# mpieva/mapAD

Measured on AMD Instinct MI355X. Metric: mapped reads/sec (50 bp, -p 0.03), higher is better.
Workload: dtype u64+f32; 1 GPU; C4: synthetic genome (3000000000 bp, n = 6000000002 BWT rows), 10000000 x 50 bp reads per GPU, -p 0.03, no-damage model; reads_per_gpu=10000000, genome_bp=3000000000, index_bytes_hbm=3000000128, batches_in_flight=2, parallelism=1 GPU, index_build=GPU suffix sorting (prefix doubling over radix sorts) + host text preparation

## Files before the change

mapad_amd/csrc/darray_core.hpp:

```cpp
#pragma once
#include "search_core.hpp"

namespace mapad {

constexpr int kMaxOffset = 15;

MAPAD_HD float d_penalty(const DevParams& P, const uint8_t* seq, const uint8_t* qual, int L, int r) {
    const int to_class = base_index(seq[r]);
    const Float4 row = sdm_row(P, L, r, qual[r], to_class);
    float v = sdm_best_mismatch(row, to_class) - sdm_optimal(row, to_class);
    const int dist = r < (L - r - 1) ? r : (L - r - 1);
    if (dist >= P.gap_dist_ends) v = f32_max(v, P.gap_extend);
    return v;
}

MAPAD_HD void ext1_any(const DevIndex& ix, uint64_t lower, uint64_t size, int k, int w, uint64_t& nl, uint64_t& ns) {
#if defined(__HIP_DEVICE_COMPILE__)
    ext1_quad(ix, lower, size, k, w, nl, ns);
#else
    (void)w;
    ext1_scalar(ix, lower, size, k, nl, ns);
#endif
}

MAPAD_HD uint32_t d_chain(const DevIndex& ix, const uint8_t* seq, int L, int split, bool left_part, int offset, const float* pen,
                          float* out, int w) {
    const int part_len = left_part ? split : L - split;
    for (int p = 0; p <= offset && p < part_len; ++p) out[p] = 0.0f;
    float z = 0.0f, m = kF32Min;
    uint64_t lower = 0, size = ix.n;
    uint32_t n_ext = 0;
    for (int i = offset; i + 1 < part_len; ++i) {
        const int r = left_part ? i : L - 1 - i;
        m = f32_max(m, pen[r]);
        const int b = base_index(seq[r]);
        uint64_t nl = 0, ns = 0;
        if (b < 4) ext1_any(ix, lower, size, left_part ? 3 - b : b, w, nl, ns);
        n_ext += 1;
        if (ns < 1) {
            z += m;
            m = kF32Min;
            lower = 0; size = ix.n;
        } else {
            lower = nl; size = ns;
        }
        out[i + 1] = z;
    }
    return n_ext;
}

MAPAD_HD uint32_t d_array_scalar(const DevIndex& ix, const DevParams& P, const uint8_t* seq, const uint8_t* qual, int L, float* pen_buf,
                                 float* chain_buf, float* d_out) {
    const int split = P.start_at_end ? L : L / 2;
    for (int r = 0; r < L; ++r) { pen_buf[r] = d_penalty(P, seq, qual, L, r); d_out[r] = 0.0f; }
    uint32_t n_ext = 0;
    for (int part = 0; part < 2; ++part) {
        const bool left = part == 0;
        const int part_len = left ? split : L - split;
        for (int o = 0; o < kMaxOffset; ++o) {
            n_ext += d_chain(ix, seq, L, split, left, o, pen_buf, chain_buf, 0);
            for (int p = 0; p < part_len; ++p) {
                float& d = d_out[(left ? 0 : split) + p];
                d = f32_min(d, chain_buf[p]);
            }
        }
    }
    return n_ext;
}

}
```

mapad_amd/csrc/mapad_amd.hip:

```cpp
#include <hip/hip_runtime.h>

#include <algorithm>
#include <atomic>
#include <cstdio>
#include <cstdlib>
#include <cstring>
#include <map>
#include <memory>
#include <mutex>
#include <new>
#include <set>
#include <stdexcept>
#include <string>
#include <type_traits>
#include <unordered_map>
#include <vector>

#include "../../include/mapad_amd.h"
#include "collapse_core.hpp"
#include "darray_core.hpp"
#include "host_index.hpp"
#include "host_index_io.hpp"
#include "host_models.hpp"
#include "host_postproc.hpp"
#include "postproc_core.hpp"
#include "text_core.hpp"
#include "damage_core.hpp"
#include "coverage_core.hpp"
#include "pileup_core.hpp"
#include "panel_core.hpp"
#include "allele_core.hpp"
#include "genotype_core.hpp"
#include "dedup_core.hpp"
#include "dscore_core.hpp"
#include "rescale_core.hpp"
#include "align_core.hpp"
#include "merge_core.hpp"
#include "mappability_core.hpp"
#include "search_core.hpp"
#include "host_tail.hpp"

using namespace mapad;

namespace mapad { namespace gpuidx { void suffix_products(const uint8_t* t_host, host::Index& ix, int device, bool verbose); void last_build_info(uint64_t out[16]); } }

namespace {

enum : uint32_t { ST_POOL_OVERFLOW = 4, ST_NO_TABLE = 8, ST_TAIL = 16  };
#if !defined(MAPAD_DEFAULT_TAIL_POPS)
#define MAPAD_DEFAULT_TAIL_POPS (1u << 20)
#endif
#if !defined(MAPAD_DEFAULT_TAIL_POPS_IDLE)
#define MAPAD_DEFAULT_TAIL_POPS_IDLE (1u << 17)
#endif
constexpr int kTiers = 2;
constexpr int kStages = 3;
constexpr int kClasses = 10;
constexpr int kKeyBins = kMaxReadLen + 2;
enum { CUR_HITS = 0, CUR_OPS = 2, CUR_POOL_OVF = 4, CUR_ERR = 5, CUR_WORK = 6, CUR_OVF = 7, CUR_GROWN = 6 + 2 * kStages, CUR_HEAVY_N = CUR_GROWN + 4 , CUR_HEAVY_WORK = CUR_GROWN + 6 ,
       CUR_HEAVY_POPS = CUR_GROWN + 8 , CUR_HPROF = CUR_GROWN + 10 , CUR_TAIL = CUR_GROWN + 26 , CUR_TAIL_DRY = CUR_GROWN + 27 ,
       CUR_TAIL_F = CUR_GROWN + 28 , CUR_TAIL_STATE = CUR_GROWN + 29 ,
       CUR_TAIL_IDLE = CUR_GROWN + 30 , CUR_COUNT = CUR_GROWN + 31 };
inline uint64_t cur64(const uint32_t* cur, int k) { return (uint64_t)cur[k] | ((uint64_t)cur[k + 1] << 32); }

struct BatchDev {
    const uint8_t* seqs;
    const uint8_t* quals;
    const uint64_t* offsets;
    uint32_t n_reads;
    float* d_arrays;
    ReadCounters* counters;
    uint32_t* status;
    uint32_t* hit_count;
    uint32_t* hit_first;
    HitRec* hits_pool;
    uint32_t* ops_pool;
    uint32_t hits_cap, ops_cap;
    uint32_t* cursors;
    uint32_t* overflow_list;
    uint32_t* sort_key;
    uint32_t* key_hist;
    uint32_t order_shift;
    uint32_t* order;
    unsigned long long* prof;
    struct HeavyItem* heavy;
    uint32_t heavy_cap;
    uint8_t* tail_ring;
    uint32_t tail_stride, tail_cap, tail_lmax;
    uint32_t tail_pops;
    const uint32_t* tail_ctl;
    uint32_t tail_backlog_max, tail_min_class;
    uint32_t tail_backlog_budget;
    uint32_t tail_continue;
    uint32_t tail_gen;
    uint32_t tail_pops_idle, tail_backlog_idle;
};

struct HeavyItem {
    uint32_t read, grown;
    SearchState st;
};
static_assert(sizeof(HeavyItem) == 72, "heavy item layout");

struct ArenaPool {
    uint8_t* base;
    uint64_t stride;
    uint64_t off_nodes, off_hits, off_hit_ops, off_scratch, off_near;
    uint32_t heap_cap, node_cap, hit_ops_cap;
    uint32_t* set_owner;
    uint32_t n_sets;
};

struct GrowPools {
    uint8_t* base[kClasses + 1];
    uint32_t* owner[kClasses + 1];
    uint64_t stride[kClasses + 1], off_nodes[kClasses + 1];
    uint64_t off_hits[kClasses + 1], off_hit_ops[kClasses + 1], off_scratch[kClasses + 1];
    uint32_t heap_cap[kClasses + 1], node_cap[kClasses + 1], count[kClasses + 1];
    uint32_t set_next_class;
    uint32_t hit_ops_cap;
    uint32_t max_waits;
    uint32_t heavy_min_class;
    uint32_t wide_copy_nodes;
    uint32_t heavy_fast;
    uint32_t heavy_max_pending;
};
constexpr uint32_t kGrownShift = 27;

template <bool NL, int TOP = kTop>
__device__ __forceinline__ ArenaT<NL, TOP> carve(const ArenaPool& ap, uint32_t slot) {
    uint8_t* b = ap.base + (uint64_t)slot * ap.stride;
    ArenaT<NL, TOP> a;
    a.heap = (MAPAD_GLOBAL HeapEntry*)(b) + 1;
    a.nodes = (MAPAD_GLOBAL Node*)(b + ap.off_nodes);
    a.hits = (MAPAD_GLOBAL HitRec*)(b + ap.off_hits);
    a.hit_ops = (MAPAD_GLOBAL uint32_t*)(b + ap.off_hit_ops);
    a.scratch = (MAPAD_GLOBAL uint16_t*)(b + ap.off_scratch);
    a.top = nullptr;
    a.heap_cap = ap.heap_cap; a.node_cap = ap.node_cap; a.hit_ops_cap = ap.hit_ops_cap;
    return a;
}

#define MAPAD_SLIM_EARLY __launch_bounds__(64)
__global__ void MAPAD_SLIM_EARLY darray_kernel(DevIndex ix, DevParams P, BatchDev B, int lmax, float* long_scratch, const uint32_t* __restrict__ dup_of) {
    extern __shared__ float lds[];
    float* pen = long_scratch ? long_scratch + (size_t)blockIdx.x * 16 * lmax : lds;
    float* chains = pen + lmax;
    __shared__ uint32_t n_ext_total;
    const int lane = threadIdx.x & 63, quad = lane >> 2, w = lane & 3;
    for (uint32_t read = blockIdx.x; read < B.n_reads; read += gridDim.x) {
        if (dup_of && dup_of[read] != read) continue;
        const uint64_t off = B.offsets[read];
        const int L = (int)(B.offsets[read + 1] - off);
        const uint8_t* seq = B.seqs + off;
        const uint8_t* qual = B.quals + off;
        float* dout = B.d_arrays + off;
        if (L > lmax || P.table_base[L] < 0) {
            if (lane == 0) {
                B.status[read] = ST_NO_TABLE; atomicOr(&B.cursors[CUR_ERR], ST_NO_TABLE); B.counters[read].e_darray = 0;
                if (B.order) { B.sort_key[read] = 0; atomicAdd(&B.key_hist[(size_t)(read >> B.order_shift) * kKeyBins], 1u); }
            }
            continue;
        }
        const int split = P.start_at_end ? L : L / 2;
        uint32_t zeros = 0;
        if (lane == 0) n_ext_total = 0;
        for (int r = lane; r < L; r += 64) pen[r] = d_penalty(P, seq, qual, L, r);
        __syncthreads();
        for (int part = 0; part < 2; ++part) {
            const bool left = part == 0;
            const int part_len = left ? split : L - split;
            if (part_len == 0) continue;
            if (quad < kMaxOffset) {
                const uint32_t n_ext = d_chain(ix, seq, L, split, left, quad, pen, chains + quad * lmax, w);
                if (w == 0) atomicAdd(&n_ext_total, n_ext);
            }
            __syncthreads();
            for (int p = lane; p < part_len; p += 64) {
                float acc = 0.0f;
#pragma unroll
                for (int o = 0; o < kMaxOffset; ++o) acc = f32_min(acc, chains[o * lmax + p]);
                dout[(left ? 0 : split) + p] = acc;
                zeros += (uint32_t)__popcll(__ballot(acc == 0.0f));
            }
            __syncthreads();
        }
        if (lane == 0) {
            B.counters[read].e_darray = n_ext_total;
            if (B.order) { B.sort_key[read] = zeros; atomicAdd(&B.key_hist[(size_t)(read >> B.order_shift) * kKeyBins + zeros], 1u); }
        }
        __syncthreads();
    }
}

__global__ void order_scan_kernel(uint32_t* hist, uint32_t n_chunks, uint32_t n_bins, const uint32_t* first) {
    if (threadIdx.x != 0 || blockIdx.x != 0) return;
    uint32_t acc = first ? *first : 0u;
    for (uint32_t ch = 0; ch < n_chunks; ++ch) {
        uint32_t* h = hist + (size_t)ch * kKeyBins;
        for (int k = (int)n_bins - 1; k >= 0; --k) { const uint32_t c = h[k]; h[k] = acc; acc += c; }
    }
}
#define MAPAD_SLIM __launch_bounds__(64)
__global__ void MAPAD_SLIM order_scatter_kernel(BatchDev B, const uint32_t* __restrict__ dup_of) {
    const uint32_t lane = threadIdx.x & 63u;
    const uint32_t i = blockIdx.x * 64u + lane;
    const bool act = i < B.n_reads && (!dup_of || dup_of[i] == i);
    const uint32_t key = act ? B.sort_key[i] : 0xFFFFFFFFu;
    uint32_t* hist = B.key_hist + (size_t)((blockIdx.x * 64u) >> B.order_shift) * kKeyBins;
    uint64_t todo = __ballot(act);
    while (todo) {
        const int leader = __ffsll((long long)todo) - 1;
        const uint32_t k = (uint32_t)__builtin_amdgcn_readlane((int)key, leader);
        const bool mine = act && key == k;
        const uint64_t m = __ballot(mine);
        uint32_t base = 0;
        if ((int)lane == leader) base = atomicAdd(&hist[k], (uint32_t)__popcll(m));
        base = (uint32_t)__builtin_amdgcn_readlane((int)base, leader);
        if (mine) B.order[base + (uint32_t)__popcll(m & ((1ull << lane) - 1ull))] = i;
        todo &= ~m;
    }
}

enum { CS_GROUPS = 0, CS_TWIN_REPS = 1, CS_COLLISIONS = 2, CS_LIST = 3, CS_POPS = 4 , CS_COUNT = 8 };
struct CollapseDev {
    const uint8_t* seqs; const uint8_t* quals; const uint64_t* offsets;
    uint32_t n_reads, ignore_qual;
    collapse::Table tab;
    uint64_t* keys;
    uint32_t* dup_of;
    uint32_t* has_dup;
    uint32_t* stats;
};
struct CollapseAtomics {
    static __device__ __forceinline__ uint64_t cas64(uint64_t* p, uint64_t expected, uint64_t desired) { return (uint64_t)atomicCAS((unsigned long long*)p, (unsigned long long)expected, (unsigned long long)desired); }
    static __device__ __forceinline__ void max32(uint32_t* p, uint32_t v) { atomicMax(p, v); }
};
__global__ void MAPAD_SLIM collapse_insert_kernel(CollapseDev Q) {
    const uint32_t lane = threadIdx.x & 63u, w = lane & 3u;
    const uint32_t i = blockIdx.x * 16u + (lane >> 2);
    const bool act = i < Q.n_reads;
    uint64_t part = 0;
    int L = 0;
    if (act) {
        const uint64_t off = Q.offsets[i];
        L = (int)(Q.offsets[i + 1] - off);
        part = collapse::key_partial(Q.seqs + off, Q.quals + off, L, Q.ignore_qual != 0, (int)w, 4);
    }
    part += __shfl_xor(part, 1); part += __shfl_xor(part, 2);
    if (act && w == 0) {
        const uint64_t key = collapse::key_finish(part, L);
        Q.keys[i] = key;
        collapse::table_insert<CollapseAtomics>(Q.tab, key, i);
    }
}
__global__ void MAPAD_SLIM collapse_match_kernel(CollapseDev Q) {
    const uint32_t lane = threadIdx.x & 63u, w = lane & 3u;
    const uint32_t i = blockIdx.x * 16u + (lane >> 2);
    const bool act = i < Q.n_reads;
    uint32_t cand = i;
    bool same = true;
    if (act) {
        cand = collapse::table_find(Q.tab, Q.keys[i], i);
        if (cand != i) {
            const uint64_t off = Q.offsets[i], off_c = Q.offsets[cand];
            const int L = (int)(Q.offsets[i + 1] - off);
            same = (int)(Q.offsets[cand + 1] - off_c) == L &&
                   collapse::equal_partial(Q.seqs + off, Q.quals + off, Q.seqs + off_c, Q.quals + off_c, L, Q.ignore_qual != 0, (int)w, 4);
        }
    }
    const uint64_t agree = __ballot(same);
    same = ((agree >> (lane & ~3u)) & 0xFull) == 0xFull;
// ... 1372 lines not shown

#if !defined(MAPAD_KTOP2)
#define MAPAD_KTOP2 31
#endif
template <int LPR> struct top_of { static constexpr int value = LPR == 2 ? MAPAD_KTOP2 : kTop; };
template <int LPR, bool CONT, int PASS, bool NL, bool HEAVY, bool BWD = false>
__global__ void __launch_bounds__(64, (LPR == 1 && NL) ? 1 : LPR == 2 ? 2 : MAPAD_MIN_WAVES) search_kernel(DevIndex ix, DevParams P, BatchDev B0, ArenaPool AP0, const GrowPools* GP, uint32_t near_stride, uint32_t near_lmax, int stage) {
    const int lane = threadIdx.x & 63, w0 = lane & (LPR - 1);
    const int tier0 = stage;
    const uint32_t n_items = tier0 == 0 ? B0.n_reads : B0.cursors[CUR_OVF + 2 * (tier0 - 1)];
    if (n_items == 0) return;
    uint32_t* const cursors = B0.cursors;
    const uint32_t set = acquire_set(AP0);
    const uint32_t slot = set * (64 / LPR) + (lane / LPR);
    constexpr int TOPK = top_of<LPR>::value;
    static_assert(!HEAVY || LPR == 4, "reads are handed to heavy wavefronts by quads only");
    static_assert(!BWD || (LPR == 4 && !HEAVY), "the backward-only step is built for the default quads only");
    ArenaT<NL, TOPK> A = carve<NL, TOPK>(AP0, slot);
    extern __shared__ __attribute__((aligned(16))) uint8_t near_lds[];
    using NearBytes = typename near_ptr<uint8_t, NL>::type;
    NearBytes near;
    if constexpr (NL) near = (NearBytes)near_lds + (size_t)(lane / LPR) * near_stride;
    else near = AP0.base + (uint64_t)slot * AP0.stride + AP0.off_near;
    A.top = (typename near_ptr<HeapEntry, NL>::type)near + 1;
    const NearBytes near_qc = near + (TOPK + 1) * sizeof(HeapEntry);
    const typename near_ptr<float, NL>::type near_d = (typename near_ptr<float, NL>::type)(near_qc + ((2 * near_lmax + 15) & ~15u));
    uint32_t* work = &cursors[CUR_WORK + 2 * tier0];
    const DeviceGrow<LPR, NL, TOPK> grow{GP, &cursors[CUR_GROWN], slot, w0, stage + 2 < kStages || HEAVY, false, B0.tail_min_class};
    const uint32_t wide_copy_nodes = GP->wide_copy_nodes;
    const uint32_t tail_lo = B0.tail_pops_idle;
    bool tail_denied = false;
    bool drained = false;
#if defined(MAPAD_PROFILE_SECTIONS)
    if (lane < 2 * PROF_N + 2) g_prof_lds[lane] = 0;
    g_prof_hist[lane] = 0;
    if (lane == 0) g_prof_lds[2 * PROF_N] = __builtin_amdgcn_s_memtime();
#endif
    bool have = false, done = false;
    ReadInT<NL> rd{near_qc, near_d, 0, 0.0f, 0};
    if constexpr (LPR == 4) rd.lane_less = w0 == 0 ? ix.less[1] : w0 == 1 ? ix.less[2] : w0 == 2 ? ix.less[3] : ix.less[4];
    if constexpr (LPR == 2) { rd.lane_less = w0 == 0 ? ix.less[1] : ix.less[3]; rd.lane_less1 = w0 == 0 ? ix.less[2] : ix.less[4]; }
    SearchState st;
#if MAPAD_NODE_PREFETCH
    NodePrefetch node_pf;
#endif
    uint32_t read = 0;
    for (;;) {
        int w = w0, tier = tier0;
#if MAPAD_OPAQUE_LANE
        asm volatile("" : "+v"(w));
        asm volatile("" : "+s"(tier));
#endif
        MAPAD_MARK(PROF_LOOP);
        if (!have && !done) {
            uint32_t item = 0;
            if (w == 0 && !drained) item = atomicAdd(work, 1u);
            item = group_bcast<LPR>(item);
            uint32_t again = ~0u;
            if (PASS == 0 && !HEAVY && (drained | (item >= n_items))) {
                drained = true;
                if (w == 0) {
                    const uint32_t cnt = __hip_atomic_load(&cursors[CUR_OVF], __ATOMIC_RELAXED, __HIP_MEMORY_SCOPE_AGENT);
                    uint32_t cur = __hip_atomic_load(&cursors[CUR_WORK + 2], __ATOMIC_RELAXED, __HIP_MEMORY_SCOPE_AGENT);
                    while (cur < cnt) {
                        const uint32_t old = atomicCAS(&cursors[CUR_WORK + 2], cur, cur + 1u);
                        if (old == cur) { again = cur; break; }
                        cur = old;
                    }
                }
                again = group_bcast<LPR>(again);
            }
            if ((item >= n_items || drained) && again == ~0u) done = true;
            else {
                const BatchDev B = kernarg_reload(kArgOffB, B0);
                const uint32_t* items = B.overflow_list + (size_t)(tier > 0 ? tier - 1 : 0) * B.n_reads;
                if (again != ~0u) {
                    uint32_t e = 0;
                    if (w == 0) { while ((e = atomicExch(&B.overflow_list[again], 0u)) == 0u) __builtin_amdgcn_s_sleep(8); }
                    read = group_bcast<LPR>(e) - 1u;
                } else {
                    read = tier == 0 ? (B.order ? B.order[item] : item) : items[item] - 1u;
                    if (tier >= 1 && w == 0) B.overflow_list[(size_t)(tier - 1) * B.n_reads + item] = 0u;
                }
                const uint64_t off = B.offsets[read];
                rd.L = (int)(B.offsets[read + 1] - off);
                const DevParams Pf = kernarg_reload(kArgOffP, P);
                rd.thr = Pf.reject_thr[rd.L];
                rd.table = Pf.table_base[rd.L];
                if (tier == 0 && B.status[read] == ST_NO_TABLE) {
                    if (w == 0) { B.hit_count[read] = 0; B.hit_first[read] = 0; }
                } else {
                    read_setup(B.seqs + off, B.quals + off, B.d_arrays + off, rd.L, near_qc, near_d, w, LPR);
                    SearchState tmp;
                    A.n_waits = again != ~0u ? kRestarted : 0u;
                    search_init(kernarg_reload(0, ix).n, BWD ? rd.L : alignment_start_of(P, rd.L), rd, A, tmp);
                    st = tmp;
#if MAPAD_NODE_PREFETCH
                    node_pf.ok = false;
#endif
                    have = true;
                    tail_denied = false;
                }
                drain_memory();
            }
        }
        MAPAD_MARK(PROF_SETUP);
        if (__all(done)) break;
        if constexpr (PASS != 1 && LPR == 4) {
            const bool need = have && (st.heap_len != 0) & (st.status == ST_OK) & ((st.tree_len + kStepNodes > A.node_cap) | (st.heap_len + kStepNodes > A.heap_cap)) &
                              (st.tree_entries >= wide_copy_nodes);
            if (MAPAD_UNLIKELY(__any(need))) { grow.wide(A, st, lane, need); drain_memory(); }
        }
        if (have) {
            bool cont;
            DevParams Ps = P;
#if MAPAD_OPAQUE_LANE
            if constexpr (BWD) asm volatile("" : "+s"(Ps.nq), "+s"(Ps.bound_kind), "+s"(Ps.gap_dist_ends), "+s"(Ps.max_num_gaps_open), "+s"(Ps.stack_limit_abort));
            else asm volatile("" : "+s"(Ps.nq), "+s"(Ps.bound_kind), "+s"(Ps.gap_dist_ends), "+s"(Ps.max_num_gaps_open), "+s"(Ps.start_at_end), "+s"(Ps.stack_limit_abort));
#endif
#if MAPAD_NODE_PREFETCH
            if constexpr (PASS != 1 && LPR == 4 && NL) cont = search_step_pf<LPR, CONT, NL, false, BWD>(ix, Ps, rd, A, st, w, grow, node_pf);
            else
#endif
            if constexpr (PASS != 1) cont = search_step<LPR, CONT, NL, false, BWD>(ix, Ps, rd, A, st, w, grow);
            else cont = search_step<LPR, CONT, NL, false, BWD>(ix, Ps, rd, A, st, w, NoGrow());
            MAPAD_MARK(PROF_TAIL);
            auto give_to_host = [&](int why, uint32_t limit) -> int {
                const BatchDev B = kernarg_reload(kArgOffB, B0);
                if (B.tail_cap == 0) return 2;
                uint32_t k = 0xFFFFFFFEu;
                if (w == 0) {
                    if (limit == 0xFFFFFFFFu) k = atomicAdd(&cursors[CUR_TAIL], 1u);
                    else {
                        const uint32_t seen = __hip_atomic_load(B.tail_ctl + 1, __ATOMIC_RELAXED, __HIP_MEMORY_SCOPE_SYSTEM);
                        const uint32_t pend = __hip_atomic_load(B.tail_ctl, __ATOMIC_RELAXED, __HIP_MEMORY_SCOPE_SYSTEM);
                        uint32_t cur = __hip_atomic_load(&cursors[CUR_TAIL], __ATOMIC_RELAXED, __HIP_MEMORY_SCOPE_AGENT);
                        for (;;) {
                            if (cur >= B.tail_cap) { k = 0xFFFFFFFFu; break; }
                            if ((uint64_t)pend + (cur > seen ? cur - seen : 0u) >= limit) break;
                            const uint32_t old = atomicCAS(&cursors[CUR_TAIL], cur, cur + 1u);
                            if (old == cur) { k = cur; break; }
                            cur = old;
                        }
                    }
                }
                k = group_bcast<LPR>(k);
                if (k >= B.tail_cap) return k == 0xFFFFFFFEu ? 1 : 2;
                const bool with_state = PASS != 1 && TOPK == kTop && B.tail_continue != 0 && A.grown != 0 && st.n_hits == 0 && st.status == ST_OK;
                hand_to_host<LPR, NL>(B, rd, A, st, read, k, w, with_state);
                if (w == 0 && why) atomicAdd(&cursors[why], 1u);
                if (with_state) {
                    if (w == 0) atomicAdd(&cursors[CUR_TAIL_STATE], 1u);
                    const ArenaT<NL, TOPK> base = carve<NL, TOPK>(kernarg_reload(kArgOffAP, AP0), slot);
                    A.heap = base.heap; A.nodes = base.nodes; A.heap_cap = base.heap_cap; A.node_cap = base.node_cap; A.grown = 0;
                }
                return 0;
            };
// ... 169 lines not shown
    ArenaPool ap{};
    auto align = [](uint64_t x) { return (x + 127) & ~127ull; };
    ap.heap_cap = heap_cap; ap.node_cap = node_cap; ap.hit_ops_cap = hit_ops_cap;
    uint64_t o = align(heap_bytes(heap_cap));
    ap.off_nodes = o; o = align(o + (uint64_t)node_cap * sizeof(Node));
    ap.off_hits = o; o = align(o + (uint64_t)kMaxHits * sizeof(HitRec));
    ap.off_hit_ops = o; o = align(o + (uint64_t)hit_ops_cap * 4);
    ap.off_scratch = o; o = align(o + 2ull * (lmax + 1) * 2);
    ap.off_near = o; o = align(o + near_bytes(lmax));
    ap.stride = o;
    return ap;
}

}

namespace {
int zero_async(hipStream_t st, void* p, size_t bytes) {
    const uint64_t n = bytes / 4;
    if (!n) return MAPAD_OK;
    const uint32_t grid = (uint32_t)std::min<uint64_t>((n + 255) / 256, 4096);
    hipLaunchKernelGGL(zero_words_kernel, dim3(grid), dim3(64), 0, st, (uint32_t*)p, n);
    HIP_TRY(hipGetLastError());
    return MAPAD_OK;
}
int read_back_words(hipStream_t st, const void* d_src, PinnedBuf<uint32_t>& h, size_t word_off, uint32_t n_words) {
    hipLaunchKernelGGL(publish_words_kernel, dim3(1), dim3(64), 0, st, (const uint32_t*)d_src, h.data() + word_off, n_words);
    HIP_TRY(hipGetLastError());
    HIP_TRY(hipStreamSynchronize(st));
    return MAPAD_OK;
}
}

constexpr int kMaxDepth = 16;
enum Stage { ST_DEDUP, ST_DSCORE, ST_RESCALE, ST_DAMAGE, ST_COVERAGE, ST_PILEUP, ST_ALLELE, ST_GENOTYPE, ST_PANEL, ST_COUNT };
struct SlotStage {
    uint64_t gen = 0;
    DevEvent ev[2];
    bool untimed = false;
};
struct StageSums {
    uint64_t batches = 0;
    double ms = 0.0;
};
struct BatchSlot {
    hipStream_t stream = nullptr;
    bool own_stream = false;
    DevEvent ev[4];
    DevEvent ev_in;
    DevBuf<uint8_t> d_seqs, d_quals;
    DevBuf<uint64_t> d_offsets;
    DevBuf<float> d_darr, d_dscratch;
    DevBuf<ReadCounters> d_counters;
    DevBuf<uint32_t> d_status, d_hit_count, d_hit_first, d_ops, d_cursors, d_overflow, d_sort_key, d_key_hist, d_order;
    DevBuf<HitRec> d_hits;
    DevBuf<HeavyItem> d_heavy;
    DevBuf<uint64_t> d_c_hit_begin, d_c_ops_begin;
    DevBuf<unsigned long long> d_c_tiles;
    DevBuf<HitRec> d_c_hits;
    DevBuf<uint32_t> d_c_ops;
    uint64_t c_n_hits = 0, c_n_ops = 0;
    bool compacted = false;
    BatchDev last{};
    uint64_t last_total_bases = 0;
    uint32_t last_lmax = 0;
    uint32_t launch_info[8] = {0, 0, 0, 0, 0, 0, 0, 0};
    bool ev_valid = false, timed = true;
    uint64_t gen = 0;
    CoherentBuf tail_ring;
    uint32_t tail_ring_stride = 0, tail_ring_gen = 0;
    const uint8_t* tail_ring_base = nullptr;
    std::shared_ptr<std::atomic<bool>> tail_launched;
    bool tail_failed = false;
    std::shared_ptr<host::TailBatch> tail;
    DevBuf<uint8_t> d_tail_up;
    PinnedBuf<uint32_t> h_small;
    PinnedBuf<uint8_t> h_tail_stage;
    DevBuf<CoordRec> d_rec_coords;
    DevBuf<DevRecord> d_rec_out;
    DevBuf<char> d_rec_text;
    DevBuf<float> d_rec_pairs;
    DevBuf<uint32_t> d_dup_of, d_c_zeroed;
    DevBuf<uint64_t> d_c_keys;
    DevEvent ev_c[4];
    bool collapsed = false, fan_done = false, fan_d = false;
    uint32_t* c_stats = nullptr;
    SlotStage st[ST_COUNT];
    DevBuf<uint64_t> d_dd_keys;
    DevBuf<uint8_t> d_dup;
    DevBuf<int32_t> d_ds_score;
    DevBuf<uint8_t> d_ds_scored, d_ds_skip;
    DevBuf<uint8_t> d_rs_quals;
    DevBuf<AlignIn> d_an_in;
    DevBuf<uint32_t> d_an_cigar;
    DevBuf<uint8_t> d_an_md, d_an_cls;
    bool aligned = false;
    uint64_t tail_info[16] = {};

    void release() {
        d_seqs.release(); d_quals.release(); d_offsets.release(); d_darr.release(); d_dscratch.release(); d_counters.release(); d_status.release(); d_hit_count.release();
        d_hit_first.release(); d_ops.release(); d_cursors.release(); d_overflow.release(); d_sort_key.release(); d_key_hist.release(); d_order.release();
        d_hits.release(); d_heavy.release();
        d_c_hit_begin.release(); d_c_ops_begin.release(); d_c_tiles.release(); d_c_hits.release(); d_c_ops.release();
        if (tail) { host::tail_cancel(tail); tail.reset(); }
        d_tail_up.release();
        d_dup_of.release(); d_c_zeroed.release(); d_c_keys.release(); c_stats = nullptr; collapsed = false;
        for (auto& e : ev_c) e.reset();
        for (auto& s : st) { for (auto& e : s.ev) e.reset(); s.untimed = false; s.gen = 0; }
        d_dd_keys.release(); d_dup.release(); d_ds_score.release(); d_ds_scored.release(); d_ds_skip.release(); d_rs_quals.release();
        d_an_in.release(); d_an_cigar.release(); d_an_md.release(); d_an_cls.release(); aligned = false;
        d_rec_coords.release(); d_rec_out.release(); d_rec_text.release(); d_rec_pairs.release();
        for (auto& e : ev) e.reset(); ev_in.reset();
        if (own_stream && stream) (void)hipStreamDestroy(stream);
        stream = nullptr; own_stream = false;
    }
};

struct PanelDef {
    std::vector<uint64_t> slot_x;
    std::vector<uint32_t> slot_of_row;
    std::vector<uint8_t> alleles;
    bool operator==(const PanelDef& o) const { return slot_x == o.slot_x && slot_of_row == o.slot_of_row && alleles == o.alleles; }
};

struct mapad_ctx {
    int device = 0;
    hipStream_t stream = nullptr;
    mapad_params_t params{};
    const mapad_index* index = nullptr;
    host::HostTables tables;
    bool tables_dirty = true;
    std::shared_ptr<const host::HostTables> tables_snap;
    uint32_t tail_pops = 0;
    DevBuf<uint64_t> d_blocks;
    DevBuf<float> d_sdm, d_thr;
    DevBuf<int32_t> d_base;
    DevIndex dix{};
    DevParams dprm{};
    bool fetch_d = true;
    bool collapse = false;
    StageSums st[ST_COUNT];
    DevEvent ev_sum[2];
    int damage_mode = 0;
    DevBuf<unsigned long long> d_damage;
    int coverage_mode = 0;
    DevBuf<int32_t> d_cov_diff;
    DevBuf<unsigned long long> d_cov_cnt;
    DevBuf<uint32_t> d_cov_flag;
    DevBuf<CoverageSeg> d_cov_segs;
    DevBuf<long long> d_cov_sums;
    uint32_t cov_seg = 0;
    uint64_t cov_n_segs = 0;
    DevBuf<uint32_t> d_cov_win;
    DevBuf<int32_t> d_cov_tmp;
// ... 638 lines not shown
    HIP_TRY(hipStreamCreateWithFlags(out, hipStreamNonBlocking));
    return MAPAD_OK;
}

void drop_tail(mapad_ctx* c, BatchSlot& S);
int acquire_slot(mapad_ctx* c, int k) {
    BatchSlot& S = c->bs[k];
    if (S.ev_valid) { HIP_TRY(hipStreamSynchronize(S.stream)); int rc = record_times(c, S); if (rc) return rc; }
    drop_tail(c, S);
    if (c->depth == 1) S.stream = c->stream;
    else if (!S.stream) { const int rc_s = create_slot_stream(c, &S.stream); if (rc_s) return rc_s; S.own_stream = true; }
    if (c->depth > 1) {
        if (S.ev_in.ensure(hipEventDisableTiming)) return MAPAD_ERR_DEVICE;
        HIP_TRY(hipEventRecord(S.ev_in, c->stream));
        HIP_TRY(hipStreamWaitEvent(S.stream, S.ev_in, 0));
    }
    c->cur = k; c->view = k;
    return MAPAD_OK;
}

uint32_t order_shift_for(uint64_t n_reads) {
    return std::min<uint32_t>(std::max<uint32_t>(env_u32("MAPAD_ORDER_CHUNK_LOG2", n_reads >= (4u << 20) ? 21 : 20), 10), 31);
}

uint64_t collapse_table_slots(uint64_t n_reads) { uint64_t t = 64; while (t < 2 * n_reads) t <<= 1; return t; }
size_t collapse_zeroed_words(uint64_t n_reads) { return (size_t)CS_COUNT + (size_t)((n_reads + 1) & ~1ull) + 3 * (size_t)collapse_table_slots(n_reads); }

int ensure_batch_buffers(mapad_ctx* c, BatchSlot& S, uint64_t n_reads, uint64_t total_bases, uint32_t lmax, bool host_inputs) {
    int rc;
    if ((rc = upload_tables(c))) return rc;
    if ((rc = ensure_arenas(c, S, lmax, n_reads))) return rc;
    const size_t nr = std::max<uint64_t>(n_reads, 1);
    if (host_inputs) {
        if ((rc = S.d_seqs.ensure(std::max<uint64_t>(total_bases, 1)))) return rc;
        if ((rc = S.d_quals.ensure(std::max<uint64_t>(total_bases, 1)))) return rc;
        if ((rc = S.d_offsets.ensure(n_reads + 1))) return rc;
    }
    if ((rc = S.d_darr.ensure(std::max<uint64_t>(total_bases, 1)))) return rc;
    if ((rc = S.d_counters.ensure(nr))) return rc;
    if ((rc = S.d_status.ensure(nr))) return rc;
    if ((rc = S.d_hit_count.ensure(nr))) return rc;
    if ((rc = S.d_hit_first.ensure(nr))) return rc;
    {
        const uint32_t* before = S.d_overflow.p;
        if ((rc = S.d_overflow.ensure(nr * kStages))) return rc;
        if (S.d_overflow.p != before) HIP_TRY(hipMemsetAsync(S.d_overflow.p, 0, S.d_overflow.cap * sizeof(uint32_t), S.stream));
    }
    const uint32_t order_shift = order_shift_for(nr);
    const uint32_t n_chunks = (uint32_t)((nr + (1ull << order_shift) - 1) >> order_shift);
    if (env_u32("MAPAD_ORDER", 1) != 0) {
        if ((rc = S.d_sort_key.ensure(nr))) return rc;
        if ((rc = S.d_order.ensure(nr))) return rc;
        if ((rc = S.d_key_hist.ensure((size_t)n_chunks * kKeyBins))) return rc;
    }
    if (c->collapse) {
        if ((rc = S.d_order.ensure(nr))) return rc;
        if ((rc = S.d_dup_of.ensure(nr))) return rc;
        if ((rc = S.d_c_keys.ensure(nr))) return rc;
        if ((rc = S.d_c_zeroed.ensure(collapse_zeroed_words(nr)))) return rc;
    }
    if ((rc = S.d_cursors.ensure(CUR_COUNT))) return rc;
    if ((rc = S.d_heavy.ensure(2 * (size_t)c->heavy_cap))) return rc;
    const size_t hits_cap = std::max(S.d_hits.cap, (size_t)env_u32("MAPAD_HIT_POOL", (uint32_t)std::min<size_t>(2 * nr + 1024, 0xFFFFFFFFu)));
    const size_t ops_cap = std::max(S.d_ops.cap, hits_cap * (size_t)(std::min<uint32_t>(lmax, 256) + 8));
    if ((rc = S.d_hits.ensure(hits_cap))) return rc;
    if ((rc = S.d_ops.ensure(ops_cap))) return rc;
    return MAPAD_OK;
}

bool release_tail_arena(mapad_ctx* c, uint32_t grown, hipStream_t st) {
    const uint32_t cls = (grown >> kGrownShift) - 1, idx = grown & ((1u << kGrownShift) - 1);
    if (cls > (uint32_t)kClasses || idx >= c->grow.count[cls]) return false;
    hipLaunchKernelGGL(zero_words_kernel, dim3(1), dim3(64), 0, st, c->grow.owner[cls] + idx, (uint64_t)1);
    return hipGetLastError() == hipSuccess;
}
hipStream_t thread_stream(int dev) {
    static thread_local hipStream_t streams[16] = {};
    if (dev < 0 || dev >= 16) return nullptr;
    if (!streams[dev] && hipStreamCreateWithFlags(&streams[dev], hipStreamNonBlocking) != hipSuccess) streams[dev] = nullptr;
    return streams[dev];
}
bool fetch_tail_state(mapad_ctx* c, uint32_t grown, uint32_t heap_len, uint32_t tree_entries, HeapEntry* heap_phys, Node* nodes) {
    if (hipSetDevice(c->device) != hipSuccess) return false;
    const uint32_t cls = (grown >> kGrownShift) - 1, idx = grown & ((1u << kGrownShift) - 1);
    if (cls > (uint32_t)kClasses || idx >= c->grow.count[cls]) return false;
    std::unique_lock<std::mutex> g(c->tail_mu, std::defer_lock);
    hipStream_t st = nullptr;
    if (env_u32("MAPAD_TAIL_THREAD_STREAMS", 0) != 0) st = thread_stream(c->device);
    else {
        g.lock();
        if (!c->tail_stream && hipStreamCreateWithFlags(&c->tail_stream, hipStreamNonBlocking) != hipSuccess) return false;
        st = c->tail_stream;
    }
    if (!st) return false;
    const uint8_t* b = c->grow.base[cls] + (uint64_t)idx * c->grow.stride[cls];
    if (!heap_phys || !nodes) {
        (void)release_tail_arena(c, grown, st);
        (void)hipStreamSynchronize(st);
        return false;
    }
    bool ok = heap_len < c->grow.heap_cap[cls] + 8 && tree_entries <= c->grow.node_cap[cls];
    ok = ok && hipMemcpyAsync(heap_phys, b, ((size_t)HeapLayout<kTop>::phys_end(heap_len) + 1) * sizeof(HeapEntry), hipMemcpyDeviceToHost, st) == hipSuccess;
    ok = ok && hipMemcpyAsync(nodes, b + c->grow.off_nodes[cls], (size_t)tree_entries * sizeof(Node), hipMemcpyDeviceToHost, st) == hipSuccess;
    const bool released = release_tail_arena(c, grown, st);
    ok = (hipStreamSynchronize(st) == hipSuccess) && ok && released;
    return ok;
}

void drop_tail(mapad_ctx* c, BatchSlot& S) {
    if (!S.tail) return;
    std::shared_ptr<host::TailBatch> tb = S.tail;
    S.tail.reset();
    host::tail_cancel(tb);
    if (!tb->fetch_state || hipSetDevice(c->device) != hipSuccess) return;
    std::lock_guard<std::mutex> g(c->tail_mu);
    if (!c->tail_stream && hipStreamCreateWithFlags(&c->tail_stream, hipStreamNonBlocking) != hipSuccess) return;
    bool any = false;
    for (uint32_t k = 0; k < tb->cap; ++k) {
        const uint8_t* rec = tb->ring + (size_t)k * tb->stride;
        if (reinterpret_cast<const host::TailRecord*>(rec)->ready != tb->gen || tb->fetched[k]) continue;
        const host::TailState* ts = reinterpret_cast<const host::TailState*>(rec + host::tail_state_offset(tb->lmax));
        if (ts->grown) any = release_tail_arena(c, ts->grown, c->tail_stream) || any;
    }
    if (any) (void)hipStreamSynchronize(c->tail_stream);
}

uint64_t next_launch_serial() {
    static std::atomic<uint64_t> launch_serial{0};
    return launch_serial.fetch_add(1, std::memory_order_relaxed) + 1;
}
int launch_batch(mapad_ctx* c, BatchSlot& S, const uint8_t* d_seqs, const uint8_t* d_quals, const uint64_t* d_offsets, uint64_t n_reads, uint64_t total_bases,
                 uint32_t lmax, bool warm = false) {
    int rc;
    if ((rc = ensure_batch_buffers(c, S, n_reads, total_bases, lmax, false))) return rc;
    const size_t nr = std::max<uint64_t>(n_reads, 1);
    const bool ordered = env_u32("MAPAD_ORDER", 1) != 0;
    const uint32_t order_shift = order_shift_for(nr);
    const uint32_t n_chunks = (uint32_t)((nr + (1ull << order_shift) - 1) >> order_shift);
    if (ordered && (rc = zero_async(S.stream, S.d_key_hist.p, (size_t)n_chunks * kKeyBins * 4))) return rc;
    if ((rc = zero_async(S.stream, S.d_cursors.p, CUR_COUNT * 4))) return rc;
    if ((rc = zero_async(S.stream, S.d_status.p, nr * 4))) return rc;
    BatchDev B{};
    B.seqs = d_seqs; B.quals = d_quals; B.offsets = d_offsets; B.n_reads = (uint32_t)n_reads;
    B.d_arrays = S.d_darr.p; B.counters = S.d_counters.p; B.status = S.d_status.p;
    B.hit_count = S.d_hit_count.p; B.hit_first = S.d_hit_first.p;
    B.hits_pool = S.d_hits.p; B.ops_pool = S.d_ops.p;
    B.hits_cap = (uint32_t)std::min<size_t>(S.d_hits.cap, 0xFFFFFFFFu); B.ops_cap = (uint32_t)std::min<size_t>(S.d_ops.cap, 0xFFFFFFFFu);
    B.cursors = S.d_cursors.p; B.overflow_list = S.d_overflow.p;
    const bool collapse = c->collapse && !warm && n_reads != 0;
    B.sort_key = ordered ? S.d_sort_key.p : nullptr; B.key_hist = ordered ? S.d_key_hist.p : nullptr; B.order = ordered || collapse ? S.d_order.p : nullptr;
    B.order_shift = order_shift;
    S.collapsed = collapse; S.fan_done = false; S.fan_d = false; S.c_stats = nullptr;
    B.heavy = S.d_heavy.p; B.heavy_cap = c->heavy_cap;
#if defined(MAPAD_PROFILE_SECTIONS)
    if ((rc = c->d_prof.ensure(2 * PROF_N + 64))) return rc;
    HIP_TRY(hipMemsetAsync(c->d_prof.p, 0, (2 * PROF_N + 64) * 8, S.stream));
    B.prof = c->d_prof.p;
#endif
    B.tail_ring = nullptr; B.tail_stride = 0; B.tail_cap = 0; B.tail_lmax = 0; B.tail_pops = 0xFFFFFFFFu;
    B.tail_ctl = nullptr; B.tail_backlog_max = 0; B.tail_min_class = (uint32_t)kClasses; B.tail_continue = 0; B.tail_gen = 1; B.tail_backlog_budget = 0;
    B.tail_pops_idle = 0xFFFFFFFFu; B.tail_backlog_idle = 0;
    drop_tail(c, S);
    for (auto& x : S.tail_info) x = 0;
    S.tail_failed = false;
    if (c->tail_pops && !warm && n_reads) {
        const uint32_t tl = std::max<uint32_t>(lmax, 1);
        const uint32_t stride = host::tail_record_stride(tl);
        const uint32_t cap = (uint32_t)std::max<uint64_t>(1, std::min<uint64_t>(std::min<uint64_t>(n_reads, env_u32("MAPAD_TAIL_RING", 65536)), (1ull << 30) / stride));
        constexpr size_t kRingHeader = 64;
        if (!S.tail_ring.ensure(kRingHeader + (size_t)cap * stride)) return MAPAD_ERR_NOMEM;
        uint8_t* ring = S.tail_ring.p + kRingHeader;
        uint32_t* ctl = reinterpret_cast<uint32_t*>(S.tail_ring.p);
        ctl[0] = host::TailWorkers::instance().pending(); ctl[1] = 0;
        if (S.tail_ring_stride != stride || S.tail_ring_base != S.tail_ring.p) {
            const size_t holds = (S.tail_ring.cap - kRingHeader) / stride;
            for (size_t k = 0; k < holds; ++k) reinterpret_cast<host::TailRecord*>(ring + k * stride)->ready = 0;
            S.tail_ring_stride = stride; S.tail_ring_base = S.tail_ring.p; S.tail_ring_gen = 0;
        }
        if (++S.tail_ring_gen == 0) {
            const size_t holds = (S.tail_ring.cap - kRingHeader) / stride;
            for (size_t k = 0; k < holds; ++k) reinterpret_cast<host::TailRecord*>(ring + k * stride)->ready = 0;
            S.tail_ring_gen = 1;
        }
        auto tb = std::make_shared<host::TailBatch>();
        tb->ix = c->index->ix.view();
        tb->tables = c->tables_snap;
        tb->P = c->dprm;
        tb->P.sdm_table = tb->tables->sdm.data(); tb->P.table_base = tb->tables->table_base.data(); tb->P.reject_thr = tb->tables->reject_thr.data();
        tb->ring = ring; tb->stride = stride; tb->cap = cap; tb->lmax = tl; tb->ctl = ctl; tb->gen = S.tail_ring_gen;
        {
            auto launched = std::make_shared<std::atomic<bool>>(false);
            S.tail_launched = launched;
            const DevEvent* evp = &S.ev[3];
            tb->launch_done = [launched, evp]() { return launched->load(std::memory_order_acquire) && hipEventQuery(*evp) != hipErrorNotReady; };
        }
        B.tail_continue = env_u32("MAPAD_TAIL_CONTINUE", 1) && c->grow.heavy_min_class >= (uint32_t)kClasses ? 1u : 0u;
        tb->fetched.assign(cap, 0);
        if (B.tail_continue) tb->fetch_state = [c](uint32_t grown, uint32_t heap_len, uint32_t tree_entries, HeapEntry* heap_phys, Node* nodes) { return fetch_tail_state(c, grown, heap_len, tree_entries, heap_phys, nodes); };
        host::tail_start(tb);
        S.tail = tb;
        B.tail_ring = ring; B.tail_stride = stride; B.tail_cap = cap; B.tail_lmax = tl; B.tail_pops = c->tail_pops; B.tail_gen = S.tail_ring_gen;
        B.tail_ctl = ctl;
        B.tail_min_class = env_u32("MAPAD_TAIL_MIN_CLASS", 4);
        B.tail_backlog_max = env_u32("MAPAD_TAIL_BACKLOG", std::max(1u, host::TailWorkers::instance().size() / 2));
        B.tail_backlog_budget = env_u32("MAPAD_TAIL_BACKLOG_BUDGET", 8u * std::max(1u, host::TailWorkers::instance().size()));
        const uint32_t idle_pops = env_u32("MAPAD_TAIL_POPS_IDLE", MAPAD_DEFAULT_TAIL_POPS_IDLE);
        B.tail_pops_idle = idle_pops ? std::min(idle_pops, c->tail_pops) : c->tail_pops;
        B.tail_backlog_idle = env_u32("MAPAD_TAIL_BACKLOG_IDLE", std::max(1u, host::TailWorkers::instance().size()));
    }
    S.last = B; S.last_total_bases = total_bases; S.last_lmax = lmax; S.compacted = false;
    S.gen = next_launch_serial(); S.aligned = false;
    if (n_reads == 0 && !warm) return MAPAD_OK;
    const uint32_t lds_lmax = std::max<uint32_t>(lmax, 1);
    size_t lds_bytes = (size_t)16 * lds_lmax * sizeof(float);
    uint32_t grid_d = (uint32_t)std::min<uint64_t>(n_reads, (uint64_t)c->n_cu * 32);
    float* long_scratch = nullptr;
    if (lds_bytes > 48 * 1024) {
        grid_d = std::max<uint32_t>(1, std::min<uint32_t>(grid_d, (uint32_t)c->n_cu * 8));
        if ((rc = S.d_dscratch.ensure((size_t)grid_d * 16 * lds_lmax))) return rc;
        long_scratch = S.d_dscratch.p;
        lds_bytes = 0;
    }
    for (auto& e : S.ev) if (e.ensure()) return MAPAD_ERR_DEVICE;
    if (!warm) {
        if (!c->ev_ref) { if (c->ev_ref.ensure()) return MAPAD_ERR_DEVICE; HIP_TRY(hipEventRecord(c->ev_ref, S.stream)); c->history.clear(); }
        if (collapse) {
            for (auto& e : S.ev_c) if (e.ensure()) return MAPAD_ERR_DEVICE;
            const uint64_t slots = collapse_table_slots(n_reads);
            const size_t n_even = (size_t)((n_reads + 1) & ~1ull);
            CollapseDev Q{};
            Q.seqs = d_seqs; Q.quals = d_quals; Q.offsets = d_offsets; Q.n_reads = (uint32_t)n_reads; Q.ignore_qual = c->params.ignore_base_quality ? 1u : 0u;
            Q.stats = S.d_c_zeroed.p; Q.has_dup = Q.stats + CS_COUNT;
            Q.tab.inv_min = Q.has_dup + n_even; Q.tab.keys = (uint64_t*)(Q.tab.inv_min + slots); Q.tab.mask = slots - 1;
            Q.keys = S.d_c_keys.p; Q.dup_of = S.d_dup_of.p;
            S.c_stats = Q.stats;
            HIP_TRY(hipEventRecord(S.ev_c[0], S.stream));
            if ((rc = zero_async(S.stream, S.d_c_zeroed.p, collapse_zeroed_words(n_reads) * 4))) return rc;
            const uint32_t grid_q = (uint32_t)((n_reads + 15) / 16);
            hipLaunchKernelGGL(collapse_insert_kernel, dim3(grid_q), dim3(64), 0, S.stream, Q);
            hipLaunchKernelGGL(collapse_match_kernel, dim3(grid_q), dim3(64), 0, S.stream, Q);
            hipLaunchKernelGGL(collapse_start_kernel, dim3(1), dim3(64), 0, S.stream, Q.stats, B.cursors, (uint32_t)n_reads);
            if (!ordered) hipLaunchKernelGGL(collapse_list_kernel, dim3((uint32_t)((n_reads + 63) / 64)), dim3(64), 0, S.stream, (const uint32_t*)S.d_dup_of.p, Q.stats, S.d_order.p, (uint32_t)n_reads);
            HIP_TRY(hipGetLastError());
            HIP_TRY(hipEventRecord(S.ev_c[1], S.stream));
        }
        const uint32_t* dup_of = collapse ? S.d_dup_of.p : nullptr;
        HIP_TRY(hipEventRecord(S.ev[0], S.stream));
        BatchDev Bd = B;
        if (!ordered) Bd.order = nullptr;
        hipLaunchKernelGGL(darray_kernel, dim3(grid_d), dim3(64), lds_bytes, S.stream, c->dix, c->dprm, Bd, (int)lds_lmax, long_scratch, dup_of);
        HIP_TRY(hipGetLastError());
    }
    if (ordered && !warm) {
        const uint32_t* dup_of = collapse ? S.d_dup_of.p : nullptr;
        hipLaunchKernelGGL(order_scan_kernel, dim3(1), dim3(64), 0, S.stream, S.d_key_hist.p, n_chunks, std::min<uint32_t>(lmax + 2, kKeyBins), collapse ? (const uint32_t*)(B.cursors + CUR_WORK) : nullptr);
        hipLaunchKernelGGL(order_scatter_kernel, dim3((uint32_t)((n_reads + 63) / 64)), dim3(64), 0, S.stream, B, dup_of);
        HIP_TRY(hipGetLastError());
    }
    if (!warm) HIP_TRY(hipEventRecord(S.ev[1], S.stream));
    const uint32_t rpw = 64 / c->lpr;
    const uint32_t near_lmax = std::max<uint32_t>(lmax, 1);
    const uint32_t near_top = c->lpr == 2 ? MAPAD_KTOP2 : kTop;
    const bool near_fits = c->lpr == 4 ? near_lmax <= kMaxLdsReadLen : c->lpr == 2 ? (size_t)near_bytes(near_lmax, near_top) * 32 <= 65536 : (size_t)near_bytes(near_lmax) * 64 <= 65536;
    const uint32_t near_stride = (near_fits && env_u32("MAPAD_NEAR_LDS", 1)) ? near_bytes(near_lmax, near_top) : 0;
    size_t lds = (size_t)near_stride * rpw;
    {
        const size_t cu_lds = 160 * 1024;
        if (lds) {
            const size_t fit = cu_lds / lds;
            size_t per_cu = cu_lds - fit * lds < (size_t)env_u32("MAPAD_LDS_FREE_KB", 12) * 1024 ? fit - 1 : fit;
            per_cu = std::min<size_t>(per_cu, env_u32("MAPAD_SEARCH_BLOCKS_PER_CU", 32));
            if (per_cu >= 1 && per_cu < fit) lds = (cu_lds / (per_cu + 1) + 256) & ~(size_t)255;
        }
    }
    const bool cont = c->dprm.bound_kind == BOUND_CONTINUOUS;
    const bool heavy_on = c->grow.heavy_min_class < (uint32_t)kClasses;
    (void)heavy_on;
    const bool bwd = step_is_backward_only(c->dprm) && !c->general_direction;
#if defined(MAPAD_HEAVY_KERNEL)
#define MAPAD_LAUNCH(L, C, P, N)                                                                                                                                   \
    if (heavy_on && L == 4) hipLaunchKernelGGL((search_kernel<L, C, P, N, (L == 4)>), dim3(grid), dim3(64), lds, S.stream, c->dix, c->dprm, B, ap, c->d_grow.p, near_stride, near_lmax, stage); \
    else if (bwd && L == 4) hipLaunchKernelGGL((search_kernel<L, C, P, N, false, (L == 4)>), dim3(grid), dim3(64), lds, S.stream, c->dix, c->dprm, B, ap, c->d_grow.p, near_stride, near_lmax, stage); \
    else hipLaunchKernelGGL((search_kernel<L, C, P, N, false>), dim3(grid), dim3(64), lds, S.stream, c->dix, c->dprm, B, ap, c->d_grow.p, near_stride, near_lmax, stage)
#else
#define MAPAD_LAUNCH(L, C, P, N)                                                                                                                                   \
    if (bwd && L == 4) hipLaunchKernelGGL((search_kernel<L, C, P, N, false, (L == 4)>), dim3(grid), dim3(64), lds, S.stream, c->dix, c->dprm, B, ap, c->d_grow.p, near_stride, near_lmax, stage); \
    else hipLaunchKernelGGL((search_kernel<L, C, P, N, false>), dim3(grid), dim3(64), lds, S.stream, c->dix, c->dprm, B, ap, c->d_grow.p, near_stride, near_lmax, stage)
#endif
#define MAPAD_LAUNCH_PASS(P)                                                                                      \
    if (c->lpr == 2 && near_stride) { if (!cont) { MAPAD_LAUNCH(2, false, P, true); } else { MAPAD_LAUNCH(2, true, P, true); } }   \
    else if (c->lpr == 2) { if (!cont) { MAPAD_LAUNCH(2, false, P, false); } else { MAPAD_LAUNCH(2, true, P, false); } }          \
    else if (c->lpr == 4 && near_stride) { if (!cont) { MAPAD_LAUNCH(4, false, P, true); } else { MAPAD_LAUNCH(4, true, P, true); } }   \
    else if (c->lpr == 4) { if (!cont) { MAPAD_LAUNCH(4, false, P, false); } else { MAPAD_LAUNCH(4, true, P, false); } }          \
    else if (near_stride) { if (!cont) { MAPAD_LAUNCH(1, false, P, true); } else { MAPAD_LAUNCH(1, true, P, true); } }              \
    else { if (!cont) { MAPAD_LAUNCH(1, false, P, false); } else { MAPAD_LAUNCH(1, true, P, false); } }
    bool others_running = false;
    for (auto& o : c->bs) if (&o != &S && o.ev_valid && hipEventQuery(o.ev[3]) == hipErrorNotReady) others_running = true;
    const bool serialize = env_u32("MAPAD_SERIALIZE_SEARCH", n_reads >= (4u << 20) ? 1 : 0) != 0;
    if (serialize && others_running && !warm) {
        for (auto& o : c->bs) if (&o != &S && o.ev_valid) HIP_TRY(hipStreamWaitEvent(S.stream, o.ev[3], 0));
        others_running = false;
    }
    const uint32_t full_waves = c->resident_waves, shared_waves = std::max<uint32_t>(1, std::min<uint32_t>(full_waves, env_u32("MAPAD_SHARED_WAVES_PER_CU", 8) * (uint32_t)(c->depth > 1 ? c->n_cu - c->reserved_cus : c->n_cu)));
// ... 2652 lines not shown
```

Before: 3.302 million reads/s.

## Precompute packed launch records in sort order and specialize darray address spaces

The order scatter kernel now also writes a packed 16-byte record (read id, length, no-table flag, offset) at each sorted position. With four lanes per read, the search kernel fetches that record with one vector load instead of chasing order[], offsets[] and status[] through dependent global loads when it starts a read. Separately, darray_kernel is templated on whether scratch lives in global memory or LDS, so pointers carry explicit address spaces and the compiler can emit LDS or global instructions directly instead of generic flat accesses. The cost is an extra record buffer and more writes in the scatter kernel.

```diff
diff --git a/mapad_amd/csrc/darray_core.hpp b/mapad_amd/csrc/darray_core.hpp
--- a/mapad_amd/csrc/darray_core.hpp
+++ b/mapad_amd/csrc/darray_core.hpp
@@ -5,7 +5,8 @@
 
 constexpr int kMaxOffset = 15;
 
-MAPAD_HD float d_penalty(const DevParams& P, const uint8_t* seq, const uint8_t* qual, int L, int r) {
+template <class SeqPtr = const uint8_t*>
+MAPAD_HD float d_penalty(const DevParams& P, SeqPtr seq, SeqPtr qual, int L, int r) {
     const int to_class = base_index(seq[r]);
     const Float4 row = sdm_row(P, L, r, qual[r], to_class);
     float v = sdm_best_mismatch(row, to_class) - sdm_optimal(row, to_class);
@@ -23,8 +24,9 @@
 #endif
 }
 
-MAPAD_HD uint32_t d_chain(const DevIndex& ix, const uint8_t* seq, int L, int split, bool left_part, int offset, const float* pen,
-                          float* out, int w) {
+template <class SeqPtr = const uint8_t*, class PenPtr = const float*, class OutPtr = float*>
+MAPAD_HD uint32_t d_chain(const DevIndex& ix, SeqPtr seq, int L, int split, bool left_part, int offset, PenPtr pen,
+                          OutPtr out, int w) {
     const int part_len = left_part ? split : L - split;
     for (int p = 0; p <= offset && p < part_len; ++p) out[p] = 0.0f;
     float z = 0.0f, m = kF32Min;
diff --git a/mapad_amd/csrc/launch_core.hpp b/mapad_amd/csrc/launch_core.hpp
--- /dev/null
+++ b/mapad_amd/csrc/launch_core.hpp
@@ -0,0 +1,31 @@
+#pragma once
+#include <cstdint>
+
+#include "common.hpp"
+
+namespace mapad {
+
+struct LaunchRec {
+    uint32_t read, len;
+    uint64_t off;
+};
+static_assert(sizeof(LaunchRec) == 16 && alignof(LaunchRec) == 8, "launch record layout");
+
+constexpr uint32_t kLaunchLenMask = 0x7FFFu;
+constexpr uint32_t kLaunchNoTable = 0x80000000u;
+
+MAPAD_HD LaunchRec launch_pack(uint32_t read, uint32_t L, bool no_table, uint64_t off) {
+    LaunchRec r;
+    r.read = read;
+    r.len = (L & kLaunchLenMask) | (no_table ? kLaunchNoTable : 0u);
+    r.off = off;
+    return r;
+}
+MAPAD_HD void launch_unpack(const LaunchRec& r, uint32_t& read, int& L, bool& no_table, uint64_t& off) {
+    read = r.read;
+    L = (int)(r.len & kLaunchLenMask);
+    no_table = (r.len & kLaunchNoTable) != 0u;
+    off = r.off;
+}
+
+}
diff --git a/mapad_amd/csrc/mapad_amd.hip b/mapad_amd/csrc/mapad_amd.hip
--- a/mapad_amd/csrc/mapad_amd.hip
+++ b/mapad_amd/csrc/mapad_amd.hip
@@ -19,6 +19,7 @@
 #include "../../include/mapad_amd.h"
 #include "collapse_core.hpp"
 #include "darray_core.hpp"
+#include "launch_core.hpp"
 #include "host_index.hpp"
 #include "host_index_io.hpp"
 #include "host_models.hpp"
@@ -82,6 +83,7 @@
     uint32_t* key_hist;
     uint32_t order_shift;
     uint32_t* order;
+    LaunchRec* launch_rec;
     unsigned long long* prof;
     struct HeavyItem* heavy;
     uint32_t heavy_cap;
@@ -142,19 +144,23 @@
 }
 
 #define MAPAD_SLIM_EARLY __launch_bounds__(64)
+template <bool LONG>
 __global__ void MAPAD_SLIM_EARLY darray_kernel(DevIndex ix, DevParams P, BatchDev B, int lmax, float* long_scratch, const uint32_t* __restrict__ dup_of) {
     extern __shared__ float lds[];
-    float* pen = long_scratch ? long_scratch + (size_t)blockIdx.x * 16 * lmax : lds;
-    float* chains = pen + lmax;
+    using FloatPtr = typename std::conditional<LONG, MAPAD_GLOBAL float*, MAPAD_LDS float*>::type;
+    FloatPtr pen;
+    if constexpr (LONG) pen = (MAPAD_GLOBAL float*)long_scratch + (size_t)blockIdx.x * 16 * lmax;
+    else pen = (MAPAD_LDS float*)lds;
+    const FloatPtr chains = pen + lmax;
     __shared__ uint32_t n_ext_total;
     const int lane = threadIdx.x & 63, quad = lane >> 2, w = lane & 3;
     for (uint32_t read = blockIdx.x; read < B.n_reads; read += gridDim.x) {
         if (dup_of && dup_of[read] != read) continue;
         const uint64_t off = B.offsets[read];
         const int L = (int)(B.offsets[read + 1] - off);
-        const uint8_t* seq = B.seqs + off;
-        const uint8_t* qual = B.quals + off;
-        float* dout = B.d_arrays + off;
+        const MAPAD_GLOBAL uint8_t* seq = (const MAPAD_GLOBAL uint8_t*)B.seqs + off;
+        const MAPAD_GLOBAL uint8_t* qual = (const MAPAD_GLOBAL uint8_t*)B.quals + off;
+        MAPAD_GLOBAL float* dout = (MAPAD_GLOBAL float*)B.d_arrays + off;
         if (L > lmax || P.table_base[L] < 0) {
             if (lane == 0) {
                 B.status[read] = ST_NO_TABLE; atomicOr(&B.cursors[CUR_ERR], ST_NO_TABLE); B.counters[read].e_darray = 0;
@@ -207,6 +213,8 @@
     const uint32_t i = blockIdx.x * 64u + lane;
     const bool act = i < B.n_reads && (!dup_of || dup_of[i] == i);
     const uint32_t key = act ? B.sort_key[i] : 0xFFFFFFFFu;
+    LaunchRec rec{};
+    if (act && B.launch_rec) { const uint64_t off = B.offsets[i]; rec = launch_pack(i, (uint32_t)(B.offsets[i + 1] - off), B.status[i] == ST_NO_TABLE, off); }
     uint32_t* hist = B.key_hist + (size_t)((blockIdx.x * 64u) >> B.order_shift) * kKeyBins;
     uint64_t todo = __ballot(act);
     while (todo) {
@@ -217,7 +225,11 @@
         uint32_t base = 0;
         if ((int)lane == leader) base = atomicAdd(&hist[k], (uint32_t)__popcll(m));
         base = (uint32_t)__builtin_amdgcn_readlane((int)base, leader);
-        if (mine) B.order[base + (uint32_t)__popcll(m & ((1ull << lane) - 1ull))] = i;
+        if (mine) {
+            const uint32_t pos = base + (uint32_t)__popcll(m & ((1ull << lane) - 1ull));
+            B.order[pos] = i;
+            if (B.launch_rec) B.launch_rec[pos] = rec;
+        }
         todo &= ~m;
     }
 }
@@ -1696,10 +1708,24 @@
         asm volatile("" : "+s"(tier));
 #endif
         MAPAD_MARK(PROF_LOOP);
-        if (!have && !done) {
+        constexpr bool kRecords = LPR == 4;
+        auto claim = [&]() __attribute__((always_inline)) -> uint32_t {
             uint32_t item = 0;
             if (w == 0 && !drained) item = atomicAdd(work, 1u);
-            item = group_bcast<LPR>(item);
+            return item;
+        };
+        auto fetch_record = [&](uint32_t item, LaunchRec& rec) __attribute__((always_inline)) -> bool {
+            if constexpr (kRecords) {
+                const LaunchRec* recs = kernarg_reload(kArgOffB, B0).launch_rec;
+                if (tier == 0 && recs != nullptr && !drained && item < n_items) {
+                    const uint4 v = *reinterpret_cast<const uint4*>(recs + item);
+                    rec.read = v.x; rec.len = v.y; rec.off = (uint64_t)v.z | ((uint64_t)v.w << 32);
+                    return true;
+                }
+            }
+            return false;
+        };
+        auto start_read = [&](uint32_t item, bool have_rec, LaunchRec rec) __attribute__((always_inline)) {
             uint32_t again = ~0u;
             if (PASS == 0 && !HEAVY && (drained | (item >= n_items))) {
                 drained = true;
@@ -1717,21 +1743,28 @@
             if ((item >= n_items || drained) && again == ~0u) done = true;
             else {
                 const BatchDev B = kernarg_reload(kArgOffB, B0);
-                const uint32_t* items = B.overflow_list + (size_t)(tier > 0 ? tier - 1 : 0) * B.n_reads;
-                if (again != ~0u) {
-                    uint32_t e = 0;
-                    if (w == 0) { while ((e = atomicExch(&B.overflow_list[again], 0u)) == 0u) __builtin_amdgcn_s_sleep(8); }
-                    read = group_bcast<LPR>(e) - 1u;
+                uint64_t off;
+                bool no_table;
+                if (kRecords && have_rec) {
+                    launch_unpack(rec, read, rd.L, no_table, off);
                 } else {
-                    read = tier == 0 ? (B.order ? B.order[item] : item) : items[item] - 1u;
-                    if (tier >= 1 && w == 0) B.overflow_list[(size_t)(tier - 1) * B.n_reads + item] = 0u;
+                    const uint32_t* items = B.overflow_list + (size_t)(tier > 0 ? tier - 1 : 0) * B.n_reads;
+                    if (again != ~0u) {
+                        uint32_t e = 0;
+                        if (w == 0) { while ((e = atomicExch(&B.overflow_list[again], 0u)) == 0u) __builtin_amdgcn_s_sleep(8); }
+                        read = group_bcast<LPR>(e) - 1u;
+                    } else {
+                        read = tier == 0 ? (B.order ? B.order[item] : item) : items[item] - 1u;
+                        if (tier >= 1 && w == 0) B.overflow_list[(size_t)(tier - 1) * B.n_reads + item] = 0u;
+                    }
+                    off = B.offsets[read];
+                    rd.L = (int)(B.offsets[read + 1] - off);
+                    no_table = tier == 0 && B.status[read] == ST_NO_TABLE;
                 }
-                const uint64_t off = B.offsets[read];
-                rd.L = (int)(B.offsets[read + 1] - off);
                 const DevParams Pf = kernarg_reload(kArgOffP, P);
                 rd.thr = Pf.reject_thr[rd.L];
                 rd.table = Pf.table_base[rd.L];
-                if (tier == 0 && B.status[read] == ST_NO_TABLE) {
+                if (no_table) {
                     if (w == 0) { B.hit_count[read] = 0; B.hit_first[read] = 0; }
                 } else {
                     read_setup(B.seqs + off, B.quals + off, B.d_arrays + off, rd.L, near_qc, near_d, w, LPR);
@@ -1747,6 +1780,12 @@
                 }
                 drain_memory();
             }
+        };
+        if (!have && !done) {
+            const uint32_t item = group_bcast<LPR>(claim());
+            LaunchRec rec{};
+            const bool have_rec = fetch_record(item, rec);
+            start_read(item, have_rec, rec);
         }
         MAPAD_MARK(PROF_SETUP);
         if (__all(done)) break;
@@ -2022,6 +2061,7 @@
     DevBuf<float> d_darr, d_dscratch;
     DevBuf<ReadCounters> d_counters;
     DevBuf<uint32_t> d_status, d_hit_count, d_hit_first, d_ops, d_cursors, d_overflow, d_sort_key, d_key_hist, d_order;
+    DevBuf<LaunchRec> d_launch_rec;
     DevBuf<HitRec> d_hits;
     DevBuf<HeavyItem> d_heavy;
     DevBuf<uint64_t> d_c_hit_begin, d_c_ops_begin;
@@ -2068,7 +2108,7 @@
 
     void release() {
         d_seqs.release(); d_quals.release(); d_offsets.release(); d_darr.release(); d_dscratch.release(); d_counters.release(); d_status.release(); d_hit_count.release();
-        d_hit_first.release(); d_ops.release(); d_cursors.release(); d_overflow.release(); d_sort_key.release(); d_key_hist.release(); d_order.release();
+        d_hit_first.release(); d_ops.release(); d_cursors.release(); d_overflow.release(); d_sort_key.release(); d_key_hist.release(); d_order.release(); d_launch_rec.release();
         d_hits.release(); d_heavy.release();
         d_c_hit_begin.release(); d_c_ops_begin.release(); d_c_tiles.release(); d_c_hits.release(); d_c_ops.release();
         if (tail) { host::tail_cancel(tail); tail.reset(); }
@@ -2813,6 +2853,7 @@
         if ((rc = S.d_sort_key.ensure(nr))) return rc;
         if ((rc = S.d_order.ensure(nr))) return rc;
         if ((rc = S.d_key_hist.ensure((size_t)n_chunks * kKeyBins))) return rc;
+        if (env_u32("MAPAD_LAUNCH_RECORDS", 1) != 0 && (rc = S.d_launch_rec.ensure(nr))) return rc;
     }
     if (c->collapse) {
         if ((rc = S.d_order.ensure(nr))) return rc;
@@ -2911,6 +2952,7 @@
     const bool collapse = c->collapse && !warm && n_reads != 0;
     B.sort_key = ordered ? S.d_sort_key.p : nullptr; B.key_hist = ordered ? S.d_key_hist.p : nullptr; B.order = ordered || collapse ? S.d_order.p : nullptr;
     B.order_shift = order_shift;
+    B.launch_rec = ordered && !warm && c->lpr == 4 && env_u32("MAPAD_LAUNCH_RECORDS", 1) != 0 ? S.d_launch_rec.p : nullptr;
     S.collapsed = collapse; S.fan_done = false; S.fan_d = false; S.c_stats = nullptr;
     B.heavy = S.d_heavy.p; B.heavy_cap = c->heavy_cap;
 #if defined(MAPAD_PROFILE_SECTIONS)
@@ -3009,7 +3051,8 @@
         HIP_TRY(hipEventRecord(S.ev[0], S.stream));
         BatchDev Bd = B;
         if (!ordered) Bd.order = nullptr;
-        hipLaunchKernelGGL(darray_kernel, dim3(grid_d), dim3(64), lds_bytes, S.stream, c->dix, c->dprm, Bd, (int)lds_lmax, long_scratch, dup_of);
+        if (long_scratch) hipLaunchKernelGGL(darray_kernel<true>, dim3(grid_d), dim3(64), 0, S.stream, c->dix, c->dprm, Bd, (int)lds_lmax, long_scratch, dup_of);
+        else hipLaunchKernelGGL(darray_kernel<false>, dim3(grid_d), dim3(64), lds_bytes, S.stream, c->dix, c->dprm, Bd, (int)lds_lmax, long_scratch, dup_of);
         HIP_TRY(hipGetLastError());
     }
     if (ordered && !warm) {
```

Result: no change. 3.330 million reads/s, median of 6 (+0.9%).
